# NVlabs/FoundationPose

Hardware: NVIDIA H100
Metric: pose-hypotheses/sec at 640x480 RGB-D, 252 hyp, 5 refine iters (higher is better)
Workload: dtype f16

## Files before the change

### foundationpose_b200/csrc/fp_api_ops.cu

```cuda
#include "../../include/fpose.h"
#include "fp_common.cuh"
#include "fp_attn.cuh"
#include "fp_crop.cuh"
#include "fp_gemm.cuh"

#include <vector>

namespace fp {
const char* get_last_error();
int prof_collect(int kind, double* total_ms, double* total_work, int* launches);
int pose_errors_launch(const float* pts, int P, const float* pred, int N, const float* gt, int n_gt, float* add_out,
                       float* adds_out, cudaStream_t stream);
}

static int check_device_ptr(const void* p, const char* what) {
  int dev = 0;
  FP_CUDA_OK(cudaGetDevice(&dev));
  cudaPointerAttributes a;
  const cudaError_t e = cudaPointerGetAttributes(&a, p);
  if (e != cudaSuccess) {
    cudaGetLastError();
    fp::set_last_error("fp_pose_errors: %s: cudaPointerGetAttributes failed (%s)", what, cudaGetErrorString(e));
    return -1;
  }
  if (a.type != cudaMemoryTypeDevice && a.type != cudaMemoryTypeManaged) {
    fp::set_last_error("fp_pose_errors: %s is not device memory", what);
    return -1;
  }
  if (a.type == cudaMemoryTypeDevice && a.device != dev) {
    fp::set_last_error("fp_pose_errors: %s lives on device %d, the current device is %d", what, a.device, dev);
    return -1;
  }
  return 0;
}

extern "C" {

const char* fp_last_error(void) { return fp::get_last_error(); }

unsigned long long fp_launch_count(void) { return fp::launch_count(); }

int fp_prof_enable(int on) {
  fp::g_prof_on = on != 0;
  return 0;
}

int fp_prof_collect(int kind, double* total_ms, double* total_work, int* launches) {
  if (!total_ms || !total_work || !launches) {
    fp::set_last_error("fp_prof_collect: null output");
    return -1;
  }
  return fp::prof_collect(kind, total_ms, total_work, launches);
}

int fp_op_build_meshlets(int V, int F, const float* pos, const int* faces, int* info, int* face_of_tri_out,
                         float* meshlets_out) {
  try {
    if (!pos || !faces || !info || V <= 0 || F <= 0) {
      fp::set_last_error("fp_op_build_meshlets: bad argument");
      return -1;
    }
    for (int i = 0; i < 3 * F; ++i)
      if (faces[i] < 0 || faces[i] >= V) {
        fp::set_last_error("fp_op_build_meshlets: face index out of range");
        return -1;
      }
    std::vector<float> nrm((size_t)V * 3, 0.f), att((size_t)V * 3, 0.f);
    fp::MeshHost mh;
    int rc = fp::build_mesh_host(V, F, pos, nrm.data(), att.data(), 3, faces, mh);
    if (rc) return rc;
    int max_t = 0, max_v = 0, total = 0;
    for (const fp::Meshlet& m : mh.meshlets) {
      max_t = m.n_tris > max_t ? m.n_tris : max_t;
      max_v = m.n_verts > max_v ? m.n_verts : max_v;
      total += m.n_tris;
      for (int t = 0; t < m.n_tris; ++t) {
        const uint2 tr = mh.ml_tris[m.tri_off + t];
        for (int k = 0; k < 3; ++k) {
          const int slot = (tr.x >> (8 * k)) & 255;
          if (slot >= m.n_verts || mh.ml_verts[m.vert_off + slot] != faces[3 * tr.y + k]) {
            fp::set_last_error("fp_op_build_meshlets: meshlet triangle does not map back to its face");
            return -4;
          }
          const float* q = pos + 3 * faces[3 * tr.y + k];
          const float dx = q[0] - m.cx, dy = q[1] - m.cy, dz = q[2] - m.cz;
          if (dx * dx + dy * dy + dz * dz > m.r * m.r * 1.0001f + 1e-12f) {
            fp::set_last_error("fp_op_build_meshlets: vertex outside the meshlet's bounding sphere");
            return -4;
          }
        }
        if (face_of_tri_out) face_of_tri_out[m.tri_off + t] = (int)tr.y;
      }
    }
    if (meshlets_out)
      for (size_t i = 0; i < mh.meshlets.size(); ++i) {
        const fp::Meshlet& m = mh.meshlets[i];
        const float rec[8] = {m.cx, m.cy, m.cz, m.r, m.ax, m.ay, m.az, m.cutoff};
        for (int k = 0; k < 8; ++k) meshlets_out[8 * i + k] = rec[k];
      }
    info[0] = (int)mh.meshlets.size();
    info[1] = mh.closed;
    info[2] = mh.front_sign;
    info[3] = max_t;
    info[4] = max_v;
    info[5] = total;
    return 0;
  } catch (...) {
    fp::set_last_error("fp_op_build_meshlets: exception");
    return -3;
  }
}

int fp_op_attention(const void* qkv, void* out, int B, int impl, void* stream) {
  if (!qkv || !out) {
    fp::set_last_error("fp_op_attention: null argument");
    return -1;
  }
  fp::AttnParams ap;
  ap.qkv = reinterpret_cast<const __half*>(qkv);
  ap.ld = 1536;
  ap.q_off = 0;
  ap.k_off = 512;
  ap.v_off = 1024;
  ap.group_col_stride = 0;
  ap.n_groups = 1;
  ap.out = reinterpret_cast<__half*>(out);
  ap.ld_out = 512;
  ap.out_group_stride = 0;
  ap.B = B;
  ap.T = 400;
  ap.n_heads = 4;
  ap.scale = 0.08838834764831845f;
  cudaStream_t st = reinterpret_cast<cudaStream_t>(stream);
  (void)impl;
  return fp::attn_tc_launch(ap, st);
}

static fp::GemmLayer to_gemm_layer(const fp_gemm_layer_t* l) {
  fp::GemmLayer L;
  L.kind = l->kind;
  L.n_img = l->n_img;
  L.Hin = l->Hin;
  L.Win = l->Win;
  L.Cin = l->Cin;
  L.Cout = l->Cout;
  L.in = l->in;
  L.w = l->w;
  L.bias = l->bias;
  L.res = l->res;
  L.res_ld = l->res_ld;
  L.out = l->out;
  L.out_ld = l->out_ld;
  L.out_split = l->out_split;
  L.post_add = l->post_add;
  L.relu = l->relu;
  return L;
}

int fp_op_gemm_layer(const fp_gemm_layer_t* l, void* stream) {
  if (!l) {
    fp::set_last_error("fp_op_gemm_layer: null layer");
    return -1;
  }
  return fp::gemm_layer_launch(to_gemm_layer(l), reinterpret_cast<cudaStream_t>(stream));
}

int fp_op_gemm_tile_n(const fp_gemm_layer_t* l, int* tile_n) {
  if (!l || !tile_n) {
    fp::set_last_error("fp_op_gemm_tile_n: null argument");
    return -1;
  }
  return fp::gemm_layer_tile_n(to_gemm_layer(l), tile_n);
}

int fp_pose_errors(const float* pts, int P, const float* pred, int N, const float* gt, int n_gt, float* add_out,
                   float* adds_out, void* stream) {
  FP_REQUIRE(P >= 1 && P <= FP_METRICS_MAX_POINTS, "fp_pose_errors: P = %d outside [1, %d]", P, FP_METRICS_MAX_POINTS);
  FP_REQUIRE(N >= 0 && N <= FP_METRICS_MAX_POSES, "fp_pose_errors: N = %d outside [0, %d]", N, FP_METRICS_MAX_POSES);
  FP_REQUIRE(n_gt == 1 || n_gt == N, "fp_pose_errors: n_gt = %d, must be 1 or N = %d", n_gt, N);
  if (N == 0) return 0;
  FP_REQUIRE(pts && pred && gt, "fp_pose_errors: null input pointer");
  const void* ptrs[5] = {pts, pred, gt, add_out, adds_out};
  const char* names[5] = {"pts", "pred", "gt", "add_out", "adds_out"};
  for (int i = 0; i < 5; ++i)
    if (ptrs[i] && check_device_ptr(ptrs[i], names[i])) return -1;
  return fp::pose_errors_launch(pts, P, pred, N, gt, n_gt, add_out, adds_out, reinterpret_cast<cudaStream_t>(stream));
}

}
```

### foundationpose_b200/csrc/fp_gemm.cu

```cuda
#include "fp_gemm.cuh"

#include <stdarg.h>
#include <stdlib.h>
#include <string.h>

#include <mutex>
#include <vector>

#include "fp_common.cuh"
#include "fp_wgmma.cuh"

namespace fp {

static std::atomic<unsigned long long> g_launch_count{0};
static thread_local bool t_capturing = false;
void note_launches(int n) {
  if (!t_capturing) g_launch_count.fetch_add((unsigned long long)n, std::memory_order_relaxed);
}
unsigned long long launch_count() { return g_launch_count.load(std::memory_order_relaxed); }
void set_capturing(bool on) { t_capturing = on; }

std::atomic<bool> g_prof_on{false};
static std::mutex g_prof_mu;

struct ProfRec {
  cudaEvent_t e0, e1;
  double work;
  int kind;
};
static std::vector<ProfRec> g_prof_recs;

void prof_mark_begin(int kind, double work, cudaStream_t stream) {
  if (!g_prof_on) return;
  ProfRec r;
  r.kind = kind;
  r.work = work;
  cudaEventCreate(&r.e0);
  cudaEventCreate(&r.e1);
  cudaEventRecord(r.e0, stream);
  std::lock_guard<std::mutex> lk(g_prof_mu);
  g_prof_recs.push_back(r);
}
void prof_mark_end(cudaStream_t stream) {
  if (!g_prof_on) return;
  std::lock_guard<std::mutex> lk(g_prof_mu);
  if (g_prof_recs.empty()) return;
  cudaEventRecord(g_prof_recs.back().e1, stream);
}
int prof_collect(int kind, double* total_ms, double* total_work, int* launches) {
  FP_CUDA_OK(cudaDeviceSynchronize());
  std::lock_guard<std::mutex> lk(g_prof_mu);
  double ms = 0, work = 0;
  int n = 0;
  std::vector<ProfRec> keep;
  for (auto& r : g_prof_recs) {
    if (r.kind != kind) {
      keep.push_back(r);
      continue;
    }
    float t = 0.f;
    cudaEventElapsedTime(&t, r.e0, r.e1);
    ms += t;
    work += r.work;
    ++n;
    cudaEventDestroy(r.e0);
    cudaEventDestroy(r.e1);
  }
  g_prof_recs.swap(keep);
  *total_ms = ms;
  *total_work = work;
  *launches = n;
  return 0;
}

static thread_local char t_last_error[1024] = "";
void set_last_error(const char* fmt, ...) {
  va_list ap;
  va_start(ap, fmt);
  vsnprintf(t_last_error, sizeof(t_last_error), fmt, ap);
  va_end(ap);
}
const char* get_last_error() { return t_last_error; }

static thread_local int t_pdl_skip = 0;
void pdl_skip_next() { t_pdl_skip = 1; }

bool pdl_enabled() {
  if (t_pdl_skip) {
    t_pdl_skip = 0;
    return false;
  }
  static int on = -1;
  if (on < 0) {
    const char* e = getenv("FPOSE_PDL");
    on = (e && e[0] == '0') ? 0 : 1;
  }
  return on != 0;
}

struct GemmParams {
  int lg_bw, lg_bh;
  int bw, bh, bn;
  int tiles_w, tiles_h, tiles_n, n_tiles_n, total_tiles;
  int num_kb, chunks_per_tap;
  int dim_w, dim_h, dim_n;
  short tap_off[9][5];
  int Ho, Wo, n_img, Cout;
  const float* bias;
  int has_res;
  int odim_h, odim_n;
  int out_split;
  const float* post_add;
  int relu;
  double alg_flops;
};

constexpr int kBlockM = 128;
constexpr int kBlockK = 64;
constexpr int kABytes = kBlockM * kBlockK * 2;
constexpr int kTileThreads = 384;
constexpr int kSlabBytes = kBlockM * 64 * 2;
constexpr int kSmemOptIn = 232448;

constexpr int kWideSlabs = 2;
constexpr int kWideProducerRegs = 40;
constexpr int kWideConsumerRegs = 232;
template <int BN>
struct TileCfg {
  static constexpr int kBBytes = BN * kBlockK * 2;
  static constexpr int kStageBytes = kABytes + kBBytes;
  static constexpr int kBatches = BN / 64;
  static constexpr bool kAlternate = BN > 128;
  static constexpr int kSlabs = kAlternate ? kWideSlabs : kBatches;
  static constexpr int kStagingBytes = kSlabs * kSlabBytes;
  static constexpr int kRing = kSmemOptIn - kStagingBytes - 1024  - 256 ;
  static constexpr int kStages = (kRing / kStageBytes) > 8 ? 8 : (kRing / kStageBytes);
  static constexpr int kSmemBytes = kStages * kStageBytes + kStagingBytes + 1024 + 256;
  static_assert(kSmemBytes <= kSmemOptIn, "tile configuration exceeds the 227 KB opt-in shared memory");
  static_assert((2 * kStages + kSlabs) * 8 <= 256, "the mbarriers must fit their 256 bytes");
  static_assert(kBatches % kSlabs == 0, "every slab must take the same number of batches per tile");
};

template <int BN>
__global__ void __launch_bounds__(kTileThreads, 1)
    gemm_tile_kernel(const __grid_constant__ CUtensorMap map_a, const __grid_constant__ CUtensorMap map_b,
                     const __grid_constant__ CUtensorMap map_out, const __grid_constant__ CUtensorMap map_res,
                     const __grid_constant__ GemmParams p) {
  using Cfg = TileCfg<BN>;
  constexpr int S = Cfg::kStages;
  constexpr int NSLAB = Cfg::kSlabs;
  constexpr int NB = Cfg::kBatches;
  constexpr bool kAlt = Cfg::kAlternate;
  extern __shared__ uint8_t smem_raw[];
  uint8_t* smem = smem_raw + ((1024u - (smem_u32(smem_raw) & 1023u)) & 1023u);
  uint8_t* staging = smem + S * Cfg::kStageBytes;
  uint64_t* bars = reinterpret_cast<uint64_t*>(staging + Cfg::kStagingBytes);
  uint64_t* full = bars;
  uint64_t* empty = bars + S;
  uint64_t* res_full = bars + 2 * S;

  const int m_tiles = p.tiles_w * p.tiles_h * p.tiles_n;
  const int total = m_tiles * p.n_tiles_n;

  if (threadIdx.x == 0) {
    tma_prefetch_desc(&map_a);
    tma_prefetch_desc(&map_b);
    tma_prefetch_desc(&map_out);
    if (p.has_res) tma_prefetch_desc(&map_res);
    for (int s = 0; s < S; ++s) {
      mbar_init(&full[s], 1);
      mbar_init(&empty[s], 256);
    }
    for (int s = 0; s < (kAlt ? NSLAB : 1); ++s) mbar_init(&res_full[s], 1);
    mbar_fence_init();
  }
  __syncthreads();
  pdl_trigger();
  pdl_wait();

  auto decode = [&](int t, int& n_tile, int& tw, int& th, int& tn) {
    n_tile = t % p.n_tiles_n;
    const int m_tile = t / p.n_tiles_n;
    tw = m_tile % p.tiles_w;
    th = (m_tile / p.tiles_w) % p.tiles_h;
    tn = m_tile / (p.tiles_w * p.tiles_h);
  };

  if (threadIdx.x < 128) {
    if constexpr (BN > 128) regs_release<kWideProducerRegs>();
    if (threadIdx.x == 0) {
      int stage = 0, phase = 0;
      for (int t = blockIdx.x; t < total; t += gridDim.x) {
        int n_tile, tw, th, tn;
        decode(t, n_tile, tw, th, tn);
        int base[5] = {0, 0, 0, 0, 0};
        base[p.dim_w] += tw * p.bw;
        if (p.dim_h >= 0) base[p.dim_h] += th * p.bh;
        if (p.dim_n >= 0) base[p.dim_n] += tn * p.bn;
        int tap = 0, chunk = 0;
        for (int kb = 0; kb < p.num_kb; ++kb) {
          mbar_wait(&empty[stage], phase ^ 1);
          uint8_t* sa = smem + stage * Cfg::kStageBytes;
          mbar_expect_tx(&full[stage], Cfg::kStageBytes);
          tma_load_5d(&map_a, &full[stage], sa, base[0] + p.tap_off[tap][0] + chunk * kBlockK, base[1] + p.tap_off[tap][1],
                      base[2] + p.tap_off[tap][2], base[3] + p.tap_off[tap][3], base[4] + p.tap_off[tap][4]);
          tma_load_2d(&map_b, &full[stage], sa + kABytes, kb * kBlockK, n_tile * BN);
          if (++chunk == p.chunks_per_tap) {
            chunk = 0;
            ++tap;
          }
          if (++stage == S) {
            stage = 0;
            phase ^= 1;
          }
        }
      }
    }
    return;
  }

  if constexpr (BN > 128) regs_acquire<kWideConsumerRegs>();
  const int ct = threadIdx.x - 128;
  const int cw = ct >> 7;
  const int lane = threadIdx.x & 31;
  const int r0 = 64 * cw + 16 * ((ct >> 5) & 3) + (lane >> 2);
  const int cq = 2 * (lane & 3);
  const bool leader = (ct == 0);
  float acc[BN / 2];
#pragma unroll
  for (int i = 0; i < BN / 2; ++i) acc[i] = 0.f;
  int stage = 0, phase = 0, it = 0;
  for (int t = blockIdx.x; t < total; t += gridDim.x, ++it) {
    int n_tile, tw, th, tn;
    decode(t, n_tile, tw, th, tn);
    const int n0 = tn * p.bn;
    int n_o0 = n0, coff = 0;
    if (p.out_split > 0) {
      n_o0 = n0 % p.out_split;
      coff = (n0 / p.out_split) * p.Cout;
    }
    int oc[5] = {0, 0, 0, 0, 0}, rc[5] = {0, 0, 0, 0, 0};
    oc[1] = rc[1] = tw * p.bw;
    if (p.odim_h >= 0) oc[p.odim_h] = rc[p.odim_h] = th * p.bh;
    if (p.odim_n >= 0) {
      oc[p.odim_n] = n_o0;
      rc[p.odim_n] = n0;
    }
    if (leader) asm volatile("cp.async.bulk.wait_group.read 0;" ::: "memory");
    asm volatile("bar.sync 1, 256;" ::: "memory");
    if (leader && p.has_res) {
      for (int s = 0; s < NSLAB; ++s) {
        uint64_t* rb = &res_full[kAlt ? s : 0];
        if (kAlt || s == 0) mbar_expect_tx(rb, kAlt ? kSlabBytes : NSLAB * kSlabBytes);
        tma_load_5d(&map_res, rb, staging + s * kSlabBytes, n_tile * BN + s * 64, rc[1], rc[2], rc[3], rc[4]);
      }
    }

    int prev = -1;
    for (int kb = 0; kb < p.num_kb; ++kb) {
      mbar_wait(&full[stage], phase);
      const uint32_t sa = smem_u32(smem + stage * Cfg::kStageBytes);
      const uint64_t da = gmma_desc_sw128(sa + (uint32_t)cw * 8192u);
      const uint64_t db = gmma_desc_sw128(sa + kABytes);
      wgmma_fence();
#pragma unroll
      for (int k = 0; k < kBlockK / 16; ++k)
        Wgmma<BN>::ss(acc, da + (uint64_t)(2 * k), db + (uint64_t)(2 * k), (kb > 0 || k > 0) ? 1u : 0u);
      wgmma_commit();
      if (prev >= 0) {
        wgmma_wait<1>();
        mbar_arrive(&empty[prev]);
      }
      prev = stage;
      if (++stage == S) {
        stage = 0;
        phase ^= 1;
      }
    }
    const float* bias = p.bias + n_tile * BN;
    const float* pap[2] = {nullptr, nullptr};
    if (p.post_add) {
#pragma unroll
      for (int h = 0; h < 2; ++h) {
        const int row = r0 + 8 * h;
        const int jj = row & (p.bw - 1), ii = (row >> p.lg_bw) & (p.bh - 1);
        const int i = th * p.bh + ii, j = min(tw * p.bw + jj, p.Wo - 1);
        pap[h] = p.post_add + (size_t)(i * p.Wo + j) * p.Cout + n_tile * BN;
      }
    }
    float2 pe[8][2];
    auto load_pe = [&](int b) {
#pragma unroll
      for (int jl = 0; jl < 8; ++jl)
#pragma unroll
        for (int h = 0; h < 2; ++h) pe[jl][h] = __ldg(reinterpret_cast<const float2*>(pap[h] + 64 * b + 8 * jl + cq));
    };
    if (p.post_add) load_pe(0);
    wgmma_wait<0>();
    fence_regs(acc);
    if (prev >= 0) mbar_arrive(&empty[prev]);

#pragma unroll
    for (int b = 0; b < NB; ++b) {
      const int s = kAlt ? (b & 1) : b;
      uint8_t* slab = staging + s * kSlabBytes;
      if (kAlt && p.has_res && b > 0 && b + 1 < NB) {
        if (leader) {
          asm volatile("cp.async.bulk.wait_group.read 0;" ::: "memory");
          uint64_t* rb = &res_full[(b + 1) & 1];
          mbar_expect_tx(rb, kSlabBytes);
          tma_load_5d(&map_res, rb, staging + ((b + 1) & 1) * kSlabBytes, n_tile * BN + (b + 1) * 64, rc[1], rc[2],
                      rc[3], rc[4]);
        }
      }
      if (p.has_res && (kAlt || b == 0))
        mbar_wait(&res_full[kAlt ? s : 0], (uint32_t)((it * (NB / NSLAB) + b / NSLAB) & 1));
#pragma unroll
      for (int jh = 0; jh < 8; jh += 4) {
        float2 bb[4];
        __half2 rv[4][2];
#pragma unroll
        for (int jl = 0; jl < 4; ++jl) {
          bb[jl] = __ldg(reinterpret_cast<const float2*>(bias + 64 * b + 8 * (jh + jl) + cq));
          if (p.has_res) {
#pragma unroll
            for (int h = 0; h < 2; ++h) {
              const int row = r0 + 8 * h;
              rv[jl][h] = *reinterpret_cast<const __half2*>(slab + row * 128 + (((uint32_t)(jh + jl) ^ (uint32_t)(row & 7)) << 4) + cq * 2);
            }
          }
        }
#pragma unroll
        for (int jl = 0; jl < 4; ++jl) {
          const int j = 8 * b + jh + jl;
#pragma unroll
          for (int h = 0; h < 2; ++h) {
            const int row = r0 + 8 * h;
            uint32_t* cell = reinterpret_cast<uint32_t*>(slab + row * 128 + (((uint32_t)(jh + jl) ^ (uint32_t)(row & 7)) << 4) + cq * 2);
            float a0 = acc[4 * j + 2 * h] + bb[jl].x, a1 = acc[4 * j + 2 * h + 1] + bb[jl].y;
            if (p.has_res) {
              const float2 r = __half22float2(rv[jl][h]);
              a0 += r.x;
              a1 += r.y;
            }
            if (p.relu) {
              a0 = fmaxf(a0, 0.f);
              a1 = fmaxf(a1, 0.f);
            }
            if (p.post_add) {
              a0 += pe[jh + jl][h].x;
              a1 += pe[jh + jl][h].y;
            }
            *cell = pack_half2(a0, a1);
          }
        }
      }
      if (p.post_add && b + 1 < NB) load_pe(b + 1);
      if (kAlt || b == NB - 1) {
        asm volatile("fence.proxy.async.shared::cta;" ::: "memory");
        if (kAlt && leader) asm volatile("cp.async.bulk.wait_group.read 0;" ::: "memory");
        asm volatile("bar.sync 1, 256;" ::: "memory");
        if (leader) {
          for (int q = kAlt ? s : 0; q < (kAlt ? s + 1 : NSLAB); ++q)
            tma_store_5d(&map_out, staging + q * kSlabBytes, coff + n_tile * BN + (kAlt ? 64 * b : 64 * q), oc[1],
                         oc[2], oc[3], oc[4]);
          asm volatile("cp.async.bulk.commit_group;" ::: "memory");
        }
      }
    }
  }
  if (leader) asm volatile("cp.async.bulk.wait_group 0;" ::: "memory");
}

static int g_num_sms = 0;

typedef CUresult (*EncodeTiledFn)(CUtensorMap*, CUtensorMapDataType, cuuint32_t, void*, const cuuint64_t*,
                                  const cuuint64_t*, const cuuint32_t*, const cuuint32_t*,
                                  CUtensorMapInterleave, CUtensorMapSwizzle, CUtensorMapL2promotion,
                                  CUtensorMapFloatOOBfill);

static EncodeTiledFn get_encode_fn() {
  static EncodeTiledFn fn = nullptr;
  static std::once_flag once;
  std::call_once(once, [] {
    void* p = nullptr;
    cudaDriverEntryPointQueryResult qres;
    if (cudaGetDriverEntryPoint("cuTensorMapEncodeTiled", &p, cudaEnableDefault, &qres) == cudaSuccess &&
        qres == cudaDriverEntryPointSuccess)
      fn = reinterpret_cast<EncodeTiledFn>(p);
  });
  return fn;
}

static int encode_map(CUtensorMap* map, const void* base, int rank, const uint64_t* dims,
                      const uint64_t* strides_bytes , const uint32_t* box, bool swizzle128 = true) {
  EncodeTiledFn fn = get_encode_fn();
  FP_REQUIRE(fn != nullptr, "cuTensorMapEncodeTiled entry point not available (no CUDA driver?)");
  cuuint64_t gdim[5];
  cuuint64_t gstr[4];
  cuuint32_t bdim[5];
  cuuint32_t estr[5];
  for (int i = 0; i < rank; ++i) {
    gdim[i] = dims[i];
    bdim[i] = box[i];
    estr[i] = 1;
  }
  for (int i = 0; i < rank - 1; ++i) gstr[i] = strides_bytes[i];
  CUresult r = fn(map, CU_TENSOR_MAP_DATA_TYPE_FLOAT16, (cuuint32_t)rank, const_cast<void*>(base), gdim, gstr,
                  bdim, estr, CU_TENSOR_MAP_INTERLEAVE_NONE, swizzle128 ? CU_TENSOR_MAP_SWIZZLE_128B : CU_TENSOR_MAP_SWIZZLE_NONE,
                  CU_TENSOR_MAP_L2_PROMOTION_L2_256B, CU_TENSOR_MAP_FLOAT_OOB_FILL_NONE);
  FP_REQUIRE(r == CUDA_SUCCESS,
             "cuTensorMapEncodeTiled failed (%d): rank %d dims [%llu %llu %llu %llu %llu] box [%u %u %u %u %u]",
             (int)r, rank, (unsigned long long)dims[0], (unsigned long long)(rank > 1 ? dims[1] : 0),
             (unsigned long long)(rank > 2 ? dims[2] : 0), (unsigned long long)(rank > 3 ? dims[3] : 0),
             (unsigned long long)(rank > 4 ? dims[4] : 0), box[0], rank > 1 ? box[1] : 0, rank > 2 ? box[2] : 0,
             rank > 3 ? box[3] : 0, rank > 4 ? box[4] : 0);
  return 0;
}

int encode_map_f16(CUtensorMap* map, const void* base, int rank, const uint64_t* dims, const uint64_t* strides_bytes,
                   const uint32_t* box) {
  return encode_map(map, base, rank, dims, strides_bytes, box);
}
int encode_map_f16_linear(CUtensorMap* map, const void* base, int rank, const uint64_t* dims,
                          const uint64_t* strides_bytes, const uint32_t* box) {
  return encode_map(map, base, rank, dims, strides_bytes, box, false);
}
int num_sms() {
  if (g_num_sms == 0) {
    int dev = 0;
    if (cudaGetDevice(&dev) != cudaSuccess) return 0;
    if (cudaDeviceGetAttribute(&g_num_sms, cudaDevAttrMultiProcessorCount, dev) != cudaSuccess) return 0;
  }
  return g_num_sms;
}

static int ilog2(int v) {
  int l = 0;
  while ((1 << l) < v) ++l;
  return l;
}

template <int BN>
static int launch_bn(const CUtensorMap& ma, const CUtensorMap& mb, const CUtensorMap& mo, const CUtensorMap& mr,
                     const GemmParams& p, cudaStream_t stream) {
  using Cfg = TileCfg<BN>;
  static std::atomic<unsigned long long> attr_mask{0};
  if (!device_bit_test(attr_mask)) {
    FP_CUDA_OK(cudaFuncSetAttribute(gemm_tile_kernel<BN>, cudaFuncAttributeMaxDynamicSharedMemorySize, Cfg::kSmemBytes));
    device_bit_set(attr_mask);
  }
  const int sms = num_sms();
  FP_REQUIRE(sms > 0, "no CUDA device");
  const int grid = p.total_tiles < sms ? p.total_tiles : sms;
  prof_mark_begin(0, p.alg_flops, stream);
  FP_CUDA_OK(launch_pdl(gemm_tile_kernel<BN>, dim3(grid), dim3(kTileThreads), Cfg::kSmemBytes, stream, 1, ma, mb, mo, mr, p));
  prof_mark_end(stream);
  note_launches(1);
  FP_CUDA_OK(cudaGetLastError());
  return 0;
}

int stem_conv_launch(const GemmLayer& L, cudaStream_t stream);

static int gemm_layer_plan(const GemmLayer& L, cudaStream_t stream, int* tile_n) {
  if (L.kind == LK_CONV7_S2) {
    if (tile_n) {
      *tile_n = 64;
      return 0;
    }
    return stem_conv_launch(L, stream);
  }
  GemmParams p;
  memset(&p, 0, sizeof(p));
  CUtensorMap ma, mb;
  const uint64_t E = 2;
  int Ho, Wo, taps, ktot;
  int BN;
  uint64_t dims[5], str[4];
  uint32_t box[5];

  switch (L.kind) {
    case LK_LINEAR: {
      FP_REQUIRE(L.Cin % 64 == 0, "LINEAR: K=%d not a multiple of 64", L.Cin);
      Ho = 1;
      Wo = L.Win;
      taps = 1;
      p.chunks_per_tap = L.Cin / 64;
      p.bw = 128; p.bh = 1; p.bn = 1;
      p.dim_w = 1; p.dim_h = -1; p.dim_n = -1;
      dims[0] = L.Cin; dims[1] = L.Win; dims[2] = 1; dims[3] = 1; dims[4] = 1;
      str[0] = L.Cin * E; str[1] = str[0] * L.Win; str[2] = str[1]; str[3] = str[1];
      box[0] = 64; box[1] = 128; box[2] = 1; box[3] = 1; box[4] = 1;
      p.tiles_w = (L.Win + 127) / 128; p.tiles_h = 1; p.tiles_n = 1;
      break;
    }
    case LK_CONV3_S1: {
      FP_REQUIRE(L.Cin % 64 == 0, "CONV3_S1: Cin=%d not a multiple of 64", L.Cin);
      Ho = L.Hin; Wo = L.Win;
      taps = 9;
      p.chunks_per_tap = L.Cin / 64;
      if (Wo % 8 == 0 && Ho % 8 == 0) { p.bw = 8; p.bh = 8; p.bn = 2; }
      else if (Wo % 4 == 0 && Ho % 4 == 0) { p.bw = 4; p.bh = 4; p.bn = 8; }
      else FP_REQUIRE(false, "CONV3_S1: unsupported spatial size %dx%d", Ho, Wo);
      const uint64_t sw_ = (uint64_t)L.Cin * E, sh_ = sw_ * L.Win, sn_ = sh_ * L.Hin;
      p.dim_w = 1; p.dim_h = 2; p.dim_n = 3;
      dims[0] = L.Cin; dims[1] = L.Win; dims[2] = L.Hin; dims[3] = L.n_img; dims[4] = 1;
      str[0] = sw_; str[1] = sh_; str[2] = sn_; str[3] = sn_ * L.n_img;
      box[0] = 64; box[1] = p.bw; box[2] = p.bh; box[3] = p.bn; box[4] = 1;
      for (int r = 0; r < 3; ++r)
        for (int s = 0; s < 3; ++s) {
          p.tap_off[r * 3 + s][1] = (short)(s - 1);
          p.tap_off[r * 3 + s][2] = (short)(r - 1);
        }
      p.tiles_w = Wo / p.bw; p.tiles_h = Ho / p.bh; p.tiles_n = (L.n_img + p.bn - 1) / p.bn;
      break;
    }
    case LK_CONV3_S2: {
      FP_REQUIRE(L.Cin % 64 == 0, "CONV3_S2: Cin=%d not a multiple of 64", L.Cin);
      FP_REQUIRE(L.Hin % 2 == 0 && L.Win % 2 == 0, "CONV3_S2: odd input size");
      Ho = L.Hin / 2; Wo = L.Win / 2;
      taps = 9;
      p.chunks_per_tap = L.Cin / 64;
      if (Wo % 8 == 0 && Ho % 8 == 0) { p.bw = 8; p.bh = 8; p.bn = 2; }
      else if (Wo % 4 == 0 && Ho % 4 == 0) { p.bw = 4; p.bh = 4; p.bn = 8; }
      else FP_REQUIRE(false, "CONV3_S2: unsupported output size %dx%d", Ho, Wo);
      p.dim_w = 1; p.dim_h = 3; p.dim_n = 4;
      dims[0] = 2 * L.Cin; dims[1] = Wo; dims[2] = 2; dims[3] = Ho; dims[4] = L.n_img;
      str[0] = 2 * L.Cin * E; str[1] = (uint64_t)L.Win * L.Cin * E; str[2] = 2 * str[1];
      str[3] = (uint64_t)L.Hin * L.Win * L.Cin * E;
      box[0] = 64; box[1] = p.bw; box[2] = 1; box[3] = p.bh; box[4] = p.bn;
      for (int r = 0; r < 3; ++r)
        for (int s = 0; s < 3; ++s) {
          const int t = r * 3 + s;
          p.tap_off[t][0] = (short)((s == 1 ? 0 : 1) * L.Cin);
          p.tap_off[t][1] = (short)(s == 0 ? -1 : 0);
          p.tap_off[t][2] = (short)(r == 1 ? 0 : 1);
          p.tap_off[t][3] = (short)(r == 0 ? -1 : 0);
        }
      p.tiles_w = Wo / p.bw; p.tiles_h = Ho / p.bh; p.tiles_n = (L.n_img + p.bn - 1) / p.bn;
      break;
    }
    default:
      FP_REQUIRE(false, "unknown layer kind %d", L.kind);
  }
  ktot = taps * L.Cin;
  p.num_kb = ktot / 64;
  p.lg_bw = ilog2(p.bw);
  p.lg_bh = ilog2(p.bh);

  constexpr int kWideMinWaves = 8;
  constexpr int kWideMinKBlocks = 16;
  const int m_tiles = p.tiles_w * p.tiles_h * p.tiles_n;
  if (L.Cout % 256 == 0 && p.num_kb >= kWideMinKBlocks) {
    const int sms = num_sms();
    FP_REQUIRE(sms > 0, "no CUDA device");
    BN = (long long)m_tiles * (L.Cout / 256) >= (long long)kWideMinWaves * sms ? 256 : 128;
  } else if (L.Cout % 128 == 0) BN = 128;
  else if (L.Cout % 64 == 0) BN = 64;
  else FP_REQUIRE(false, "Cout=%d must be a multiple of 64", L.Cout);
  p.n_tiles_n = L.Cout / BN;
  p.total_tiles = p.tiles_w * p.tiles_h * p.tiles_n * p.n_tiles_n;
  p.Ho = Ho; p.Wo = Wo; p.n_img = L.n_img; p.Cout = L.Cout;
  p.bias = L.bias;
  p.has_res = L.res != nullptr;
  p.out_split = L.out_split;
  p.post_add = L.post_add;
  p.relu = L.relu;
  {
    const double k_real = (double)taps * L.Cin;
    p.alg_flops = 2.0 * (double)L.n_img * Ho * Wo * L.Cout * k_real;
  }
  FP_REQUIRE(L.out_ld % 8 == 0 && (!L.res || L.res_ld % 8 == 0), "out_ld / res_ld must be multiples of 8");
  FP_REQUIRE(L.out_split == 0 || L.out_split % p.bn == 0,
             "out_split=%d must be a multiple of the tile's image count %d (pad the A/B batch boundary)", L.out_split,
             p.bn);
  if (tile_n) {
    *tile_n = BN;
    return 0;
  }
  if (p.total_tiles == 0) return 0;

  int rc = encode_map(&ma, L.in, 5, dims, str, box);
  if (rc) return rc;
  uint64_t wd[2] = {(uint64_t)ktot, (uint64_t)L.Cout};
  uint64_t ws[1] = {(uint64_t)ktot * E};
  uint32_t wb[2] = {64, (uint32_t)BN};
  rc = encode_map(&mb, L.w, 2, wd, ws, wb);
  if (rc) return rc;
  CUtensorMap mo, mr;
  {
    uint64_t od[5], os[4];
    uint32_t ob[5];
    const bool lin = (L.kind == LK_LINEAR);
    const int n_out = L.out_split > 0 ? (L.n_img - L.out_split) : L.n_img;
    FP_REQUIRE(n_out > 0, "out_split=%d leaves no output images (n_img=%d)", L.out_split, L.n_img);
    auto fill = [&](int ld, int nimg) {
      const uint64_t sw_ = (uint64_t)ld * E, sh_ = sw_ * Wo, sn_ = sh_ * Ho;
      od[0] = (uint64_t)ld;
      ob[0] = 64;
      od[4] = 1;
      ob[4] = 1;
      if (lin) {
        od[1] = (uint64_t)Wo; od[2] = 1; od[3] = 1;
        os[0] = sw_; os[1] = sh_; os[2] = sh_; os[3] = sh_;
        ob[1] = (uint32_t)p.bw; ob[2] = 1; ob[3] = 1;
      } else {
        od[1] = (uint64_t)Wo; od[2] = (uint64_t)Ho; od[3] = (uint64_t)nimg;
        os[0] = sw_; os[1] = sh_; os[2] = sn_; os[3] = sn_ * nimg;
        ob[1] = (uint32_t)p.bw; ob[2] = (uint32_t)p.bh; ob[3] = (uint32_t)p.bn;
      }
    };
    p.odim_h = lin ? -1 : 2;
    p.odim_n = lin ? -1 : 3;
    fill(L.out_ld, n_out);
    rc = encode_map(&mo, L.out, 5, od, os, ob);
    if (rc) return rc;
    if (L.res) {
      fill(L.res_ld, L.n_img);
      rc = encode_map(&mr, L.res, 5, od, os, ob);
      if (rc) return rc;
    } else {
      mr = mo;
    }
  }
  if (BN == 256) return launch_bn<256>(ma, mb, mo, mr, p, stream);
  return BN == 128 ? launch_bn<128>(ma, mb, mo, mr, p, stream) : launch_bn<64>(ma, mb, mo, mr, p, stream);
}

int gemm_layer_launch(const GemmLayer& L, cudaStream_t stream) { return gemm_layer_plan(L, stream, nullptr); }

int gemm_layer_tile_n(const GemmLayer& L, int* tile_n) { return gemm_layer_plan(L, nullptr, tile_n); }

}
```

### foundationpose_b200/csrc/fp_gemm.cuh

```cuda
#pragma once
#include <cuda.h>
#include <cuda_runtime.h>
#include <stdint.h>

#include <atomic>

namespace fp {

enum LayerKind : int {
  LK_LINEAR = 0,
  LK_CONV3_S1 = 1,
  LK_CONV3_S2 = 2,
  LK_CONV7_S2 = 3,
};

struct GemmLayer {
  int kind;
  int n_img;
  int Hin, Win;
  int Cin;
  int Cout;
  const void* in;
  const void* w;
  const float* bias;
  const void* res;
  int res_ld;
  void* out;
  int out_ld;
  int out_split;
  const float* post_add;
  int relu;
};

int gemm_layer_launch(const GemmLayer& L, cudaStream_t stream);
int gemm_layer_tile_n(const GemmLayer& L, int* tile_n);


void prof_mark_begin(int kind, double work, cudaStream_t stream);
void prof_mark_end(cudaStream_t stream);
extern std::atomic<bool> g_prof_on;

}
```

### foundationpose_b200/ops.py

```python
import ctypes as C

import torch

from . import _lib
from ._lib import lib


def _ptr(t):
    return None if t is None else C.c_void_p(t.data_ptr())


def _stream():
    return C.c_void_p(torch.cuda.current_stream().cuda_stream)


def _require_cuda(*ts):
    for t in ts:
        if t is not None and not t.is_cuda:
            raise _lib.FposeError("libfpose operators need CUDA tensors (there is no CPU path)")


def gemm_layer(kind, x, w_packed, bias, *, n_img, Hin, Win, Cin, Cout, out=None, out_ld=None, out_split=0,
               res=None, res_ld=0, post_add=None, relu=False):
    _require_cuda(x, w_packed, bias, res, post_add, out)
    assert x.dtype == torch.float16 and w_packed.dtype == torch.float16 and bias.dtype == torch.float32
    if kind == _lib.LAYER_LINEAR:
        Ho, Wo = 1, Win
    elif kind == _lib.LAYER_CONV3_S1:
        Ho, Wo = Hin, Win
    else:
        Ho, Wo = Hin // 2, Win // 2
    if out is None:
        out_ld = Cout
        out = torch.empty(n_img, Ho, Wo, Cout, dtype=torch.float16, device=x.device)
    L = _lib.GemmLayer(kind, n_img, Hin, Win, Cin, Cout, _ptr(x), _ptr(w_packed), _ptr(bias), _ptr(res),
                       res_ld, _ptr(out), out_ld, out_split, _ptr(post_add), 1 if relu else 0)
    _lib.check(lib.fp_op_gemm_layer(C.byref(L), _stream()), "fp_op_gemm_layer")
    return out


def gemm_tile_n(kind, *, n_img, Hin, Win, Cin, Cout, out_split=0):
    lib.fp_op_gemm_tile_n.argtypes = [C.POINTER(_lib.GemmLayer), C.POINTER(C.c_int)]
    lib.fp_op_gemm_tile_n.restype = C.c_int
    L = _lib.GemmLayer(kind, n_img, Hin, Win, Cin, Cout, None, None, None, None, 0, None, Cout, out_split, None, 0)
    tile_n = C.c_int(0)
    _lib.check(lib.fp_op_gemm_tile_n(C.byref(L), C.byref(tile_n)), "fp_op_gemm_tile_n")
    return tile_n.value


lib.fp_op_attention.argtypes = [C.c_void_p, C.c_void_p, C.c_int, C.c_int, C.c_void_p]
lib.fp_op_attention.restype = C.c_int


def attention(qkv, impl=1):
    _require_cuda(qkv)
    assert qkv.dtype == torch.float16 and qkv.shape[1] == 1536 and qkv.shape[0] % 400 == 0
    B = qkv.shape[0] // 400
    out = torch.empty(qkv.shape[0], 512, dtype=torch.float16, device=qkv.device)
    _lib.check(lib.fp_op_attention(_ptr(qkv), _ptr(out), B, impl, _stream()), "fp_op_attention")
    return out
```

### include/fpose.h

```cpp
#ifndef FPOSE_H_
#define FPOSE_H_

#include <stddef.h>
#include <stdint.h>

#ifdef __cplusplus
extern "C" {
#endif

const char* fp_last_error(void);
unsigned long long fp_launch_count(void);

int fp_prof_enable(int on);
int fp_prof_collect(int kind, double* total_ms, double* total_work, int* launches);


#define FP_LAYER_LINEAR 0
#define FP_LAYER_CONV3_S1 1
#define FP_LAYER_CONV3_S2 2
#define FP_LAYER_CONV7_S2 3

typedef struct fp_gemm_layer {
  int kind;
  int n_img;
  int Hin, Win;
  int Cin;
  int Cout;
  const void* in;
  const void* w;
  const float* bias;
  const void* res;
  int res_ld;
  void* out;
  int out_ld;
  int out_split;
  const float* post_add;
  int relu;
} fp_gemm_layer_t;

int fp_op_gemm_layer(const fp_gemm_layer_t* layer, void* stream);
int fp_op_gemm_tile_n(const fp_gemm_layer_t* layer, int* tile_n);

int fp_op_attention(const void* qkv, void* out, int B, int impl, void* stream);



#define FP_METRICS_MAX_POINTS 131072
#define FP_METRICS_MAX_POSES (1 << 24)
int fp_pose_errors(const float* pts, int P, const float* pred, int N, const float* gt, int n_gt,
                   float* add_out, float* adds_out, void* stream);

typedef struct fp_ctx fp_ctx;

int fp_create(fp_ctx** ctx);
int fp_destroy(fp_ctx* ctx);

int fp_set_config(fp_ctx* ctx, int which, float crop_ratio, float rot_normalizer);

typedef struct fp_tensor {
  const char* name;
  const void* data;
  int dtype;
  long long numel;
} fp_tensor_t;

int fp_load_network(fp_ctx* ctx, int which, const fp_tensor_t* tensors, int n);

int fp_set_mesh(fp_ctx* ctx, int V, int F, const float* pos, const float* nrm, const float* uv, const float* vcol,
                const int* faces, const unsigned char* tex_rgb, int Ht, int Wt, float diameter);
#define FP_MAX_MESHES 64
int fp_set_mesh_slot(fp_ctx* ctx, int slot, int V, int F, const float* pos, const float* nrm, const float* uv,
                     const float* vcol, const int* faces, const unsigned char* tex_rgb, int Ht, int Wt, float diameter);
int fp_mesh_info(fp_ctx* ctx, int* info);

#define FP_FRAME_ON_DEVICE 1
#define FP_FRAME_FILTER_DEPTH 2
int fp_set_frame(fp_ctx* ctx, const unsigned char* rgb, const float* depth, const float* K, int H, int W, int flags,
                 float zfar, void* stream);
int fp_set_xyz_map(fp_ctx* ctx, const float* xyz, void* stream);
int fp_get_depth(fp_ctx* ctx, float* depth_out_dev, float* xyz_out_dev, void* stream);

int fp_start_poses(fp_ctx* ctx, const unsigned char* mask, int mask_on_device, const float* rot_grid, int N,
                   float* poses_out, float* info_out, void* stream);

int fp_make_crops(fp_ctx* ctx, const float* poses, int N, int mode, void* crops_out, float* dbg_out, float* win_out,
                  void* stream);
int fp_set_crop_tile(fp_ctx* ctx, int tile);
int fp_crop_stats(fp_ctx* ctx, const float* poses, int N, int mode, int* stats_out_host, void* stream);

int fp_refine(fp_ctx* ctx, const float* poses_in, int N, int iterations, float* poses_out, float* last_trans,
              float* last_rot, void* stream);

int fp_score(fp_ctx* ctx, const float* poses, int N, float* scores_out, int* best_out, void* stream);
int fp_score_features(fp_ctx* ctx, const float* poses, int N, float* feats_out, void* stream);
int fp_score_tail(fp_ctx* ctx, const float* feats, int L, float* scores_out, int* best_out, void* stream);

int fp_register(fp_ctx* ctx, const float* poses_host, int N, int iterations, float* poses_out_host,
                float* scores_out_host, int* best_out_host, void* stream);

int fp_track(fp_ctx* ctx, const unsigned char* rgb_host, const float* depth_host, const float* K, int H, int W,
             const float* pose_in_dev, int iterations, float* pose_out_dev, float* pose_out_host, void* stream);
int fp_track_objects(fp_ctx* ctx, const unsigned char* rgb_host, const float* depth_host, const float* K, int H, int W,
                     int M, const int* slots_host, const float* poses_in_dev, int iterations, float* poses_out_dev,
                     float* poses_out_host, void* stream);
#define FP_MAX_CAMERAS 16
int fp_track_cameras(fp_ctx* ctx, int C, const unsigned char* const* rgb_host, const float* const* depth_host,
                     const float* K, const int* H, const int* W, int M, const int* camera_of, const int* slots_host,
                     const float* poses_in_dev, int iterations, float* poses_out_dev, float* poses_out_host, void* stream);
int fp_register_objects(fp_ctx* ctx, const unsigned char* rgb_host, const float* depth_host, const float* K, int H, int W,
                        int M, const int* slots_host, const int* n_hyp_host, const unsigned char* masks_host,
                        const float* rot_grids_dev, int iterations, float* poses_out_dev, float* scores_out_dev,
                        int* best_out_dev, float* info_out_dev, void* stream);
int fp_register_cameras(fp_ctx* ctx, int C, const unsigned char* const* rgb_host, const float* const* depth_host,
                        const float* K, const int* H, const int* W, int M, const int* camera_of, const int* slots_host,
                        const int* n_hyp_host, const unsigned char* const* masks_host, const float* rot_grids_dev,
                        int iterations, float* poses_out_dev, float* scores_out_dev, int* best_out_dev, float* info_out_dev,
                        void* stream);
unsigned long long fp_graph_captures(fp_ctx* ctx);

int fp_vis(fp_ctx* ctx, int kind, const float* poses_a, const float* poses_b, int N, const int* order,
           unsigned char* canvas_out, int* hw_out, void* stream);
int fp_vis_size(int kind, int N, int* hw_out);
int fp_vis_colormap(unsigned char* rgb_out);
int fp_vis_crops(fp_ctx* ctx, const float* poses, int N, int mode, float* rec_out, void* stream);
unsigned long long fp_vis_workspace_bytes(fp_ctx* ctx);

typedef struct fp_group fp_group;
int fp_group_create(int ndev, const int* dev_ids, fp_group** out);
int fp_group_destroy(fp_group* g);
int fp_group_size(fp_group* g);
fp_ctx* fp_group_ctx(fp_group* g, int i);
int fp_group_load_network(fp_group* g, int which, const fp_tensor_t* tensors, int n);
int fp_group_set_config(fp_group* g, int which, float crop_ratio, float rot_normalizer);
int fp_group_set_mesh(fp_group* g, int V, int F, const float* pos, const float* nrm, const float* uv, const float* vcol,
                      const int* faces, const unsigned char* tex_rgb, int Ht, int Wt, float diameter);
int fp_group_register(fp_group* g, const unsigned char* rgb_host, const float* depth_host, const float* K, int H, int W,
                      const unsigned char* mask_host, const float* rot_grid_host, int N, int iterations,
                      float* poses_out_host, float* scores_out_host, int* best_out_host, float* info_out_host);

int fp_op_refine_net(fp_ctx* ctx, const void* crops, int N, float* trans_out, float* rot_out, void* stream);
int fp_op_score_feats(fp_ctx* ctx, const void* crops, int N, float* feats_out, void* stream);
int fp_op_tokens(fp_ctx* ctx, int which, const void* crops, int N, void* tokens_out, void* stream);
int fp_op_build_meshlets(int V, int F, const float* pos, const int* faces, int* info, int* face_of_tri_out,
                         float* meshlets_out );
int fp_op_depth_filter(const float* depth_dev, float* out_dev, int H, int W, int which, void* stream);
int fp_op_pose_update(const float* poses_in, const float* trans, const float* rot, float* poses_out, int N,
                      float mesh_diameter, float rot_normalizer, void* stream);

#ifdef __cplusplus
}
#endif
#endif
```

Measured before the change: 3611.

## Add 256-row tall GEMM tiles for Cout=128 conv layers with many tiles

Measured after the change: 3698 (median of 6 runs). +2.4%, better.

```diff
diff --git a/foundationpose_b200/csrc/fp_api_ops.cu b/foundationpose_b200/csrc/fp_api_ops.cu
--- a/foundationpose_b200/csrc/fp_api_ops.cu
+++ b/foundationpose_b200/csrc/fp_api_ops.cu
@@ -170,7 +170,17 @@
     fp::set_last_error("fp_op_gemm_tile_n: null argument");
     return -1;
   }
-  return fp::gemm_layer_tile_n(to_gemm_layer(l), tile_n);
+  int tile_m = 0;
+  return fp::gemm_layer_tile(to_gemm_layer(l), &tile_m, tile_n);
+}
+
+int fp_op_gemm_tile_m(const fp_gemm_layer_t* l, int* tile_m) {
+  if (!l || !tile_m) {
+    fp::set_last_error("fp_op_gemm_tile_m: null argument");
+    return -1;
+  }
+  int tile_n = 0;
+  return fp::gemm_layer_tile(to_gemm_layer(l), tile_m, &tile_n);
 }
 
 int fp_pose_errors(const float* pts, int P, const float* pred, int N, const float* gt, int n_gt, float* add_out,
diff --git a/foundationpose_b200/csrc/fp_gemm.cu b/foundationpose_b200/csrc/fp_gemm.cu
--- a/foundationpose_b200/csrc/fp_gemm.cu
+++ b/foundationpose_b200/csrc/fp_gemm.cu
@@ -113,11 +113,11 @@
   const float* post_add;
   int relu;
   double alg_flops;
+  int half_img;
 };
 
 constexpr int kBlockM = 128;
 constexpr int kBlockK = 64;
-constexpr int kABytes = kBlockM * kBlockK * 2;
 constexpr int kTileThreads = 384;
 constexpr int kSlabBytes = kBlockM * 64 * 2;
 constexpr int kSmemOptIn = 232448;
@@ -125,12 +125,15 @@
 constexpr int kWideSlabs = 2;
 constexpr int kWideProducerRegs = 40;
 constexpr int kWideConsumerRegs = 232;
-template <int BN>
+template <int BM, int BN>
 struct TileCfg {
+  static constexpr int kHalves = BM / kBlockM;
+  static constexpr int kABytes = BM * kBlockK * 2;
   static constexpr int kBBytes = BN * kBlockK * 2;
   static constexpr int kStageBytes = kABytes + kBBytes;
   static constexpr int kBatches = BN / 64;
-  static constexpr bool kAlternate = BN > 128;
+  static constexpr int kPasses = kHalves * kBatches;
+  static constexpr bool kAlternate = kPasses > 2;
   static constexpr int kSlabs = kAlternate ? kWideSlabs : kBatches;
   static constexpr int kStagingBytes = kSlabs * kSlabBytes;
   static constexpr int kRing = kSmemOptIn - kStagingBytes - 1024  - 256 ;
@@ -138,19 +141,22 @@
   static constexpr int kSmemBytes = kStages * kStageBytes + kStagingBytes + 1024 + 256;
   static_assert(kSmemBytes <= kSmemOptIn, "tile configuration exceeds the 227 KB opt-in shared memory");
   static_assert((2 * kStages + kSlabs) * 8 <= 256, "the mbarriers must fit their 256 bytes");
-  static_assert(kBatches % kSlabs == 0, "every slab must take the same number of batches per tile");
+  static_assert(kPasses % kSlabs == 0, "every slab must take the same number of passes per tile");
 };
 
-template <int BN>
+template <int BM, int BN>
 __global__ void __launch_bounds__(kTileThreads, 1)
     gemm_tile_kernel(const __grid_constant__ CUtensorMap map_a, const __grid_constant__ CUtensorMap map_b,
                      const __grid_constant__ CUtensorMap map_out, const __grid_constant__ CUtensorMap map_res,
                      const __grid_constant__ GemmParams p) {
-  using Cfg = TileCfg<BN>;
+  using Cfg = TileCfg<BM, BN>;
   constexpr int S = Cfg::kStages;
   constexpr int NSLAB = Cfg::kSlabs;
   constexpr int NB = Cfg::kBatches;
+  constexpr int NH = Cfg::kHalves;
+  constexpr int NP = Cfg::kPasses;
   constexpr bool kAlt = Cfg::kAlternate;
+  constexpr bool kRealloc = BM * BN > 128 * 128;
   extern __shared__ uint8_t smem_raw[];
   uint8_t* smem = smem_raw + ((1024u - (smem_u32(smem_raw) & 1023u)) & 1023u);
   uint8_t* staging = smem + S * Cfg::kStageBytes;
@@ -187,7 +193,7 @@
   };
 
   if (threadIdx.x < 128) {
-    if constexpr (BN > 128) regs_release<kWideProducerRegs>();
+    if constexpr (kRealloc) regs_release<kWideProducerRegs>();
     if (threadIdx.x == 0) {
       int stage = 0, phase = 0;
       for (int t = blockIdx.x; t < total; t += gridDim.x) {
@@ -204,7 +210,7 @@
           mbar_expect_tx(&full[stage], Cfg::kStageBytes);
           tma_load_5d(&map_a, &full[stage], sa, base[0] + p.tap_off[tap][0] + chunk * kBlockK, base[1] + p.tap_off[tap][1],
                       base[2] + p.tap_off[tap][2], base[3] + p.tap_off[tap][3], base[4] + p.tap_off[tap][4]);
-          tma_load_2d(&map_b, &full[stage], sa + kABytes, kb * kBlockK, n_tile * BN);
+          tma_load_2d(&map_b, &full[stage], sa + Cfg::kABytes, kb * kBlockK, n_tile * BN);
           if (++chunk == p.chunks_per_tap) {
             chunk = 0;
             ++tap;
@@ -219,16 +225,18 @@
     return;
   }
 
-  if constexpr (BN > 128) regs_acquire<kWideConsumerRegs>();
+  if constexpr (kRealloc) regs_acquire<kWideConsumerRegs>();
   const int ct = threadIdx.x - 128;
   const int cw = ct >> 7;
   const int lane = threadIdx.x & 31;
   const int r0 = 64 * cw + 16 * ((ct >> 5) & 3) + (lane >> 2);
   const int cq = 2 * (lane & 3);
   const bool leader = (ct == 0);
-  float acc[BN / 2];
-#pragma unroll
-  for (int i = 0; i < BN / 2; ++i) acc[i] = 0.f;
+  float acc[NH][BN / 2];
+#pragma unroll
+  for (int hh = 0; hh < NH; ++hh)
+#pragma unroll
+    for (int i = 0; i < BN / 2; ++i) acc[hh][i] = 0.f;
   int stage = 0, phase = 0, it = 0;
   for (int t = blockIdx.x; t < total; t += gridDim.x, ++it) {
     int n_tile, tw, th, tn;
@@ -246,6 +254,7 @@
       oc[p.odim_n] = n_o0;
       rc[p.odim_n] = n0;
     }
+    static_assert(NSLAB <= NB, "the passes fetched during the main loop lie in the tile's first half");
     if (leader) asm volatile("cp.async.bulk.wait_group.read 0;" ::: "memory");
     asm volatile("bar.sync 1, 256;" ::: "memory");
     if (leader && p.has_res) {
@@ -261,11 +270,14 @@
       mbar_wait(&full[stage], phase);
       const uint32_t sa = smem_u32(smem + stage * Cfg::kStageBytes);
       const uint64_t da = gmma_desc_sw128(sa + (uint32_t)cw * 8192u);
-      const uint64_t db = gmma_desc_sw128(sa + kABytes);
+      const uint64_t db = gmma_desc_sw128(sa + Cfg::kABytes);
       wgmma_fence();
 #pragma unroll
       for (int k = 0; k < kBlockK / 16; ++k)
-        Wgmma<BN>::ss(acc, da + (uint64_t)(2 * k), db + (uint64_t)(2 * k), (kb > 0 || k > 0) ? 1u : 0u);
+#pragma unroll
+        for (int hh = 0; hh < NH; ++hh)
+          Wgmma<BN>::ss(acc[hh], da + (uint64_t)(1024 * hh + 2 * k), db + (uint64_t)(2 * k),
+                        (kb > 0 || k > 0) ? 1u : 0u);
       wgmma_commit();
       if (prev >= 0) {
         wgmma_wait<1>();
@@ -278,43 +290,49 @@
       }
     }
     const float* bias = p.bias + n_tile * BN;
-    const float* pap[2] = {nullptr, nullptr};
+    const float* pap[NH][2] = {};
     if (p.post_add) {
 #pragma unroll
-      for (int h = 0; h < 2; ++h) {
-        const int row = r0 + 8 * h;
-        const int jj = row & (p.bw - 1), ii = (row >> p.lg_bw) & (p.bh - 1);
-        const int i = th * p.bh + ii, j = min(tw * p.bw + jj, p.Wo - 1);
-        pap[h] = p.post_add + (size_t)(i * p.Wo + j) * p.Cout + n_tile * BN;
-      }
+      for (int hh = 0; hh < NH; ++hh)
+#pragma unroll
+        for (int h = 0; h < 2; ++h) {
+          const int row = kBlockM * hh + r0 + 8 * h;
+          const int jj = row & (p.bw - 1), ii = (row >> p.lg_bw) & (p.bh - 1);
+          const int i = th * p.bh + ii, j = min(tw * p.bw + jj, p.Wo - 1);
+          pap[hh][h] = p.post_add + (size_t)(i * p.Wo + j) * p.Cout + n_tile * BN;
+        }
     }
     float2 pe[8][2];
-    auto load_pe = [&](int b) {
+    auto load_pe = [&](int q) {
 #pragma unroll
       for (int jl = 0; jl < 8; ++jl)
 #pragma unroll
-        for (int h = 0; h < 2; ++h) pe[jl][h] = __ldg(reinterpret_cast<const float2*>(pap[h] + 64 * b + 8 * jl + cq));
+        for (int h = 0; h < 2; ++h)
+          pe[jl][h] = __ldg(reinterpret_cast<const float2*>(pap[q / NB][h] + 64 * (q % NB) + 8 * jl + cq));
     };
     if (p.post_add) load_pe(0);
     wgmma_wait<0>();
-    fence_regs(acc);
+#pragma unroll
+    for (int hh = 0; hh < NH; ++hh) fence_regs(acc[hh]);
     if (prev >= 0) mbar_arrive(&empty[prev]);
 
 #pragma unroll
-    for (int b = 0; b < NB; ++b) {
-      const int s = kAlt ? (b & 1) : b;
+    for (int q = 0; q < NP; ++q) {
+      const int hh = q / NB, b = q % NB;
+      const int s = kAlt ? (q & 1) : q;
       uint8_t* slab = staging + s * kSlabBytes;
-      if (kAlt && p.has_res && b > 0 && b + 1 < NB) {
+      if (kAlt && p.has_res && q > 0 && q + 1 < NP) {
         if (leader) {
           asm volatile("cp.async.bulk.wait_group.read 0;" ::: "memory");
-          uint64_t* rb = &res_full[(b + 1) & 1];
+          const int qn = q + 1;
+          uint64_t* rb = &res_full[qn & 1];
           mbar_expect_tx(rb, kSlabBytes);
-          tma_load_5d(&map_res, rb, staging + ((b + 1) & 1) * kSlabBytes, n_tile * BN + (b + 1) * 64, rc[1], rc[2],
-                      rc[3], rc[4]);
-        }
-      }
-      if (p.has_res && (kAlt || b == 0))
-        mbar_wait(&res_full[kAlt ? s : 0], (uint32_t)((it * (NB / NSLAB) + b / NSLAB) & 1));
+          tma_load_5d(&map_res, rb, staging + (qn & 1) * kSlabBytes, n_tile * BN + (qn % NB) * 64, rc[1], rc[2],
+                      rc[3] + (qn / NB) * p.half_img, rc[4]);
+        }
+      }
+      if (p.has_res && (kAlt || q == 0))
+        mbar_wait(&res_full[kAlt ? s : 0], (uint32_t)((it * (NP / NSLAB) + q / NSLAB) & 1));
 #pragma unroll
       for (int jh = 0; jh < 8; jh += 4) {
         float2 bb[4];
@@ -337,7 +355,7 @@
           for (int h = 0; h < 2; ++h) {
             const int row = r0 + 8 * h;
             uint32_t* cell = reinterpret_cast<uint32_t*>(slab + row * 128 + (((uint32_t)(jh + jl) ^ (uint32_t)(row & 7)) << 4) + cq * 2);
-            float a0 = acc[4 * j + 2 * h] + bb[jl].x, a1 = acc[4 * j + 2 * h + 1] + bb[jl].y;
+            float a0 = acc[hh][4 * j + 2 * h] + bb[jl].x, a1 = acc[hh][4 * j + 2 * h + 1] + bb[jl].y;
             if (p.has_res) {
               const float2 r = __half22float2(rv[jl][h]);
               a0 += r.x;
@@ -355,15 +373,15 @@
           }
         }
       }
-      if (p.post_add && b + 1 < NB) load_pe(b + 1);
-      if (kAlt || b == NB - 1) {
+      if (p.post_add && q + 1 < NP) load_pe(q + 1);
+      if (kAlt || q == NP - 1) {
         asm volatile("fence.proxy.async.shared::cta;" ::: "memory");
         if (kAlt && leader) asm volatile("cp.async.bulk.wait_group.read 0;" ::: "memory");
         asm volatile("bar.sync 1, 256;" ::: "memory");
         if (leader) {
-          for (int q = kAlt ? s : 0; q < (kAlt ? s + 1 : NSLAB); ++q)
-            tma_store_5d(&map_out, staging + q * kSlabBytes, coff + n_tile * BN + (kAlt ? 64 * b : 64 * q), oc[1],
-                         oc[2], oc[3], oc[4]);
+          for (int u = kAlt ? s : 0; u < (kAlt ? s + 1 : NSLAB); ++u)
+            tma_store_5d(&map_out, staging + u * kSlabBytes, coff + n_tile * BN + (kAlt ? 64 * b : 64 * u),
+                         oc[1], oc[2], oc[3] + hh * p.half_img, oc[4]);
           asm volatile("cp.async.bulk.commit_group;" ::: "memory");
         }
       }
@@ -441,20 +459,20 @@
   return l;
 }
 
-template <int BN>
-static int launch_bn(const CUtensorMap& ma, const CUtensorMap& mb, const CUtensorMap& mo, const CUtensorMap& mr,
-                     const GemmParams& p, cudaStream_t stream) {
-  using Cfg = TileCfg<BN>;
+template <int BM, int BN>
+static int launch_tile(const CUtensorMap& ma, const CUtensorMap& mb, const CUtensorMap& mo, const CUtensorMap& mr,
+                       const GemmParams& p, cudaStream_t stream) {
+  using Cfg = TileCfg<BM, BN>;
   static std::atomic<unsigned long long> attr_mask{0};
   if (!device_bit_test(attr_mask)) {
-    FP_CUDA_OK(cudaFuncSetAttribute(gemm_tile_kernel<BN>, cudaFuncAttributeMaxDynamicSharedMemorySize, Cfg::kSmemBytes));
+    FP_CUDA_OK(cudaFuncSetAttribute(gemm_tile_kernel<BM, BN>, cudaFuncAttributeMaxDynamicSharedMemorySize, Cfg::kSmemBytes));
     device_bit_set(attr_mask);
   }
   const int sms = num_sms();
   FP_REQUIRE(sms > 0, "no CUDA device");
   const int grid = p.total_tiles < sms ? p.total_tiles : sms;
   prof_mark_begin(0, p.alg_flops, stream);
-  FP_CUDA_OK(launch_pdl(gemm_tile_kernel<BN>, dim3(grid), dim3(kTileThreads), Cfg::kSmemBytes, stream, 1, ma, mb, mo, mr, p));
+  FP_CUDA_OK(launch_pdl(gemm_tile_kernel<BM, BN>, dim3(grid), dim3(kTileThreads), Cfg::kSmemBytes, stream, 1, ma, mb, mo, mr, p));
   prof_mark_end(stream);
   note_launches(1);
   FP_CUDA_OK(cudaGetLastError());
@@ -463,9 +481,10 @@
 
 int stem_conv_launch(const GemmLayer& L, cudaStream_t stream);
 
-static int gemm_layer_plan(const GemmLayer& L, cudaStream_t stream, int* tile_n) {
+static int gemm_layer_plan(const GemmLayer& L, cudaStream_t stream, int* tile_m, int* tile_n) {
   if (L.kind == LK_CONV7_S2) {
     if (tile_n) {
+      *tile_m = 128;
       *tile_n = 64;
       return 0;
     }
@@ -559,6 +578,21 @@
   } else if (L.Cout % 128 == 0) BN = 128;
   else if (L.Cout % 64 == 0) BN = 64;
   else FP_REQUIRE(false, "Cout=%d must be a multiple of 64", L.Cout);
+
+  constexpr int kTallMinWaves = 8;
+  int BM = 128;
+  if (L.kind != LK_LINEAR && L.Cout == 128) {
+    const int sms = num_sms();
+    FP_REQUIRE(sms > 0, "no CUDA device");
+    const long long tall_tiles = (long long)p.tiles_w * p.tiles_h * ((L.n_img + 2 * p.bn - 1) / (2 * p.bn));
+    if (tall_tiles >= (long long)kTallMinWaves * sms) BM = 256;
+  }
+  p.half_img = p.bn;
+  if (BM == 256) {
+    p.bn *= 2;
+    box[p.dim_n] = (uint32_t)p.bn;
+    p.tiles_n = (L.n_img + p.bn - 1) / p.bn;
+  }
   p.n_tiles_n = L.Cout / BN;
   p.total_tiles = p.tiles_w * p.tiles_h * p.tiles_n * p.n_tiles_n;
   p.Ho = Ho; p.Wo = Wo; p.n_img = L.n_img; p.Cout = L.Cout;
@@ -576,6 +610,7 @@
              "out_split=%d must be a multiple of the tile's image count %d (pad the A/B batch boundary)", L.out_split,
              p.bn);
   if (tile_n) {
+    *tile_m = BM;
     *tile_n = BN;
     return 0;
   }
@@ -608,7 +643,7 @@
       } else {
         od[1] = (uint64_t)Wo; od[2] = (uint64_t)Ho; od[3] = (uint64_t)nimg;
         os[0] = sw_; os[1] = sh_; os[2] = sn_; os[3] = sn_ * nimg;
-        ob[1] = (uint32_t)p.bw; ob[2] = (uint32_t)p.bh; ob[3] = (uint32_t)p.bn;
+        ob[1] = (uint32_t)p.bw; ob[2] = (uint32_t)p.bh; ob[3] = (uint32_t)p.half_img;
       }
     };
     p.odim_h = lin ? -1 : 2;
@@ -624,12 +659,13 @@
       mr = mo;
     }
   }
-  if (BN == 256) return launch_bn<256>(ma, mb, mo, mr, p, stream);
-  return BN == 128 ? launch_bn<128>(ma, mb, mo, mr, p, stream) : launch_bn<64>(ma, mb, mo, mr, p, stream);
-}
-
-int gemm_layer_launch(const GemmLayer& L, cudaStream_t stream) { return gemm_layer_plan(L, stream, nullptr); }
-
-int gemm_layer_tile_n(const GemmLayer& L, int* tile_n) { return gemm_layer_plan(L, nullptr, tile_n); }
-
-}
+  if (BM == 256) return launch_tile<256, 128>(ma, mb, mo, mr, p, stream);
+  if (BN == 256) return launch_tile<128, 256>(ma, mb, mo, mr, p, stream);
+  return BN == 128 ? launch_tile<128, 128>(ma, mb, mo, mr, p, stream) : launch_tile<128, 64>(ma, mb, mo, mr, p, stream);
+}
+
+int gemm_layer_launch(const GemmLayer& L, cudaStream_t stream) { return gemm_layer_plan(L, stream, nullptr, nullptr); }
+
+int gemm_layer_tile(const GemmLayer& L, int* tile_m, int* tile_n) { return gemm_layer_plan(L, nullptr, tile_m, tile_n); }
+
+}
diff --git a/foundationpose_b200/csrc/fp_gemm.cuh b/foundationpose_b200/csrc/fp_gemm.cuh
--- a/foundationpose_b200/csrc/fp_gemm.cuh
+++ b/foundationpose_b200/csrc/fp_gemm.cuh
@@ -33,7 +33,7 @@
 };
 
 int gemm_layer_launch(const GemmLayer& L, cudaStream_t stream);
-int gemm_layer_tile_n(const GemmLayer& L, int* tile_n);
+int gemm_layer_tile(const GemmLayer& L, int* tile_m, int* tile_n);
 
 
 void prof_mark_begin(int kind, double work, cudaStream_t stream);
diff --git a/foundationpose_b200/ops.py b/foundationpose_b200/ops.py
--- a/foundationpose_b200/ops.py
+++ b/foundationpose_b200/ops.py
@@ -48,6 +48,15 @@
     return tile_n.value
 
 
+def gemm_tile_m(kind, *, n_img, Hin, Win, Cin, Cout, out_split=0):
+    lib.fp_op_gemm_tile_m.argtypes = [C.POINTER(_lib.GemmLayer), C.POINTER(C.c_int)]
+    lib.fp_op_gemm_tile_m.restype = C.c_int
+    L = _lib.GemmLayer(kind, n_img, Hin, Win, Cin, Cout, None, None, None, None, 0, None, Cout, out_split, None, 0)
+    tile_m = C.c_int(0)
+    _lib.check(lib.fp_op_gemm_tile_m(C.byref(L), C.byref(tile_m)), "fp_op_gemm_tile_m")
+    return tile_m.value
+
+
 lib.fp_op_attention.argtypes = [C.c_void_p, C.c_void_p, C.c_int, C.c_int, C.c_void_p]
 lib.fp_op_attention.restype = C.c_int
 
diff --git a/include/fpose.h b/include/fpose.h
--- a/include/fpose.h
+++ b/include/fpose.h
@@ -40,6 +40,7 @@
 
 int fp_op_gemm_layer(const fp_gemm_layer_t* layer, void* stream);
 int fp_op_gemm_tile_n(const fp_gemm_layer_t* layer, int* tile_n);
+int fp_op_gemm_tile_m(const fp_gemm_layer_t* layer, int* tile_m);
 
 int fp_op_attention(const void* qkv, void* out, int B, int impl, void* stream);
 
```
